# GewelsJI/MVLT

Measured on AMD Instinct MI355X. Metric: image-text pairs/sec/node, PVT-tiny MVLT pre-train step, higher is better.
Workload: dtype bf16

## Files before the change

### include/mvlt_hip.h

```cpp
#ifndef MVLT_HIP_H
#define MVLT_HIP_H
#include <stdint.h>
#ifdef __cplusplus
extern "C" {
#endif

#define MVLT_DT_BF16 0
#define MVLT_DT_FP32 1

#define MVLT_ABI_VERSION 8
const char* mvlt_last_error(void);
int mvlt_abi_version(void);
const char* mvlt_last_kernel(void);
int mvlt_sizeof(const char* name);

typedef struct mvlt_rowmap {
  int mode, rows_per_batch, batch_stride, offset;
  int r, w_in, tokens_in, hw_out, w_out, c_seg;
  int h_in;
} mvlt_rowmap;

typedef struct mvlt_gemm_nt_args {
  const void* A; const void* B; void* C;
  int M, N, K, lda, ldb, ldc;
// ... 163 lines not shown
  const void* residual;
  const float* row_scale; int rows_per_scale;
  void* out;
  void* h_out;
  float* dw1; float* db1; float* dw2; float* db2;
  int M, C, hid;
  const float* ln_x; const float* ln_gamma; const float* ln_beta; float ln_eps;
  void* ln_y; float* ln_mean; float* ln_rstd;
  void* out_op;
  const float* post_gamma; const float* post_beta; float post_eps;
  void* post_y; float* post_mean; float* post_rstd;
  const float* lnb_x; const float* lnb_mean; const float* lnb_rstd; const float* lnb_gamma;
  void* lnb_dx; void* lnb_dx2; const float* lnb_dx2_scale; int lnb_dx2_rows_per_scale;
  float* lnb_partials;
  void* partials; long partials_bytes; int defer_fold;
} mvlt_mlp_args;
int mvlt_mlp_fwd(const mvlt_mlp_args* args, void* stream);
int mvlt_mlp_bwd_dx(const mvlt_mlp_args* args, void* stream);
int mvlt_mlp_bwd_dw(const mvlt_mlp_args* args, void* stream);
int mvlt_add_column_sums(const float* in, long rows, int cols, int ld, float* dst0, int n0, float* dst1, void* stream);

int mvlt_col_stats(const float* z, int ldz, long M, int C, float* sum, float* sumsq, void* stream);
int mvlt_bn_finalize(const float* sum, const float* sumsq, int copies , long M, int C, float eps, float momentum, float* mean, float* rstd,
                     float* running_mean, float* running_var , void* stream);
int mvlt_bn_norm(const void* z, int ldz, int z_dtype, const float* mean, const float* rstd, const float* gamma, const float* beta, long M, int C,
                 void* y32, int ld32, int y32_dtype , void* y_op, int ld_op, int op_dtype , void* stream);
int mvlt_bn_finalize_norm(const void* z , int ldz, const float* sum, const float* sumsq, int copies, float eps, float momentum, float* mean, float* rstd,
                          float* running_mean, float* running_var , const float* gamma, const float* beta, long M, int C,
                          void* y32, int ld32, int y32_dtype, void* y_op , int ld_op, void* stream);
int mvlt_bn_bwd_reduce(const void* dy, int lddy, const void* z, int ldz, int z_dtype, const float* mean, const float* rstd, long M, int C,
// ... 21 lines not shown
```

### mvlt_amd/_lib.py

```python
import ctypes as C
import os

import torch

_HERE = os.path.dirname(os.path.abspath(__file__))
LIB_PATH = os.environ.get("MVLT_HIP_LIB") or os.path.join(_HERE, "libmvlt_hip.so")


class MVLTError(RuntimeError):
    pass


if not os.path.exists(LIB_PATH):
    raise ImportError(f"{LIB_PATH} is missing: build it with `python -m mvlt_amd.build` (hipcc, gfx950). "
                      "mvlt_amd has no CPU or eager fallback.")
lib = C.CDLL(LIB_PATH)

c_int, c_float, c_void_p, c_long = C.c_int, C.c_float, C.c_void_p, C.c_long


class RowMap(C.Structure):
    _fields_ = [(n, c_int) for n in ("mode", "rows_per_batch", "batch_stride", "offset",
                                     "r", "w_in", "tokens_in", "hw_out", "w_out", "c_seg", "h_in")]

# ... 58 lines not shown
                ("ldq", c_int), ("ldkv", c_int), ("ldo", c_int), ("lddkv", c_int),
                ("k_off", c_int), ("v_off", c_int), ("scale", c_float), ("dtype", c_int), ("dkv_dtype", c_int)]


class MlpArgs(C.Structure):
    _fields_ = [("x", c_void_p), ("dy", c_void_p), ("w1", c_void_p), ("wb", c_void_p), ("wc", c_void_p),
                ("b1", c_void_p), ("b2", c_void_p), ("residual", c_void_p), ("row_scale", c_void_p), ("rows_per_scale", c_int),
                ("out", c_void_p), ("h_out", c_void_p), ("dw1", c_void_p), ("db1", c_void_p), ("dw2", c_void_p), ("db2", c_void_p),
                ("M", c_int), ("C", c_int), ("hid", c_int),
                ("ln_x", c_void_p), ("ln_gamma", c_void_p), ("ln_beta", c_void_p), ("ln_eps", c_float),
                ("ln_y", c_void_p), ("ln_mean", c_void_p), ("ln_rstd", c_void_p), ("out_op", c_void_p),
                ("post_gamma", c_void_p), ("post_beta", c_void_p), ("post_eps", c_float),
                ("post_y", c_void_p), ("post_mean", c_void_p), ("post_rstd", c_void_p),
                ("lnb_x", c_void_p), ("lnb_mean", c_void_p), ("lnb_rstd", c_void_p), ("lnb_gamma", c_void_p),
                ("lnb_dx", c_void_p), ("lnb_dx2", c_void_p), ("lnb_dx2_scale", c_void_p), ("lnb_dx2_rows_per_scale", c_int),
                ("lnb_partials", c_void_p), ("partials", c_void_p), ("partials_bytes", c_long), ("defer_fold", c_int)]


STRUCTS = (("mvlt_rowmap", RowMap), ("mvlt_prep_desc", PrepDesc), ("mvlt_gemm_nt_args", GemmNTArgs), ("mvlt_gemm_tn_args", GemmTNArgs),
           ("mvlt_layernorm_args", LayerNormArgs), ("mvlt_layernorm_bwd_args", LayerNormBwdArgs),
           ("mvlt_attn_args", AttnArgs), ("mvlt_attn_bwd_args", AttnBwdArgs), ("mvlt_mlp_args", MlpArgs))

_vp, _i, _l, _f, _u64, _str = c_void_p, c_int, c_long, c_float, C.c_uint64, C.c_char_p
_by_args = lambda cls: (_i, [C.POINTER(cls), _vp])
PROTOTYPES = {
    "mvlt_last_error": (_str, []),
    "mvlt_abi_version": (_i, []),
    "mvlt_last_kernel": (_str, []),
    "mvlt_sizeof": (_i, [_str]),
    "mvlt_gemm_nt": _by_args(GemmNTArgs),
    "mvlt_gemm_tn": _by_args(GemmTNArgs),
# ... 132 lines not shown
```

### mvlt_amd/csrc/mlp.hip

```cpp
#include "common.h"
#include "../../include/mvlt_hip.h"
#include <type_traits>

namespace {

#ifndef MVLT_GELU_LUT
#define MVLT_GELU_LUT 1
#endif
#include "gelu_lut.inc"
constexpr int GELU_LUT_BYTES = MVLT_GELU_LUT_PAD * 8;
template <int NWV> __device__ __forceinline__ void gelu_lut_dma(unsigned lds_base, int wave, int lane) {
  for (int k = wave; k < GELU_LUT_BYTES / 1024; k += NWV)
    glds16((const char*)&g_gelu_lut[0][0] + k * 1024 + lane * 16, __builtin_amdgcn_readfirstlane(lds_base + k * 1024));
}
__device__ __forceinline__ unsigned gelu_lut_off(unsigned u) {
  return min(max(u, (unsigned)MVLT_GELU_LUT_BASE), (unsigned)MVLT_GELU_LUT_TOP) << 3;
}
__device__ __forceinline__ float gelu_lut_sign(float h) { return __builtin_bit_cast(float, (__builtin_bit_cast(unsigned, h) & 0x80000000u) | 0x3f800000u); }
template <int WHICH> __device__ __forceinline__ void gelu_lut_one2(const char* lut0, float h0, float h1, float& r0, float& r1) {
  const unsigned pk = __builtin_bit_cast(unsigned, __builtin_convertvector(f32x2{h0, h1}, bf16x2));
  const float t0 = *(const float*)(lut0 + gelu_lut_off(pk & 0x7fffu) + 4 * WHICH), t1 = *(const float*)(lut0 + gelu_lut_off((pk >> 16) & 0x7fffu) + 4 * WHICH);
  r0 = __builtin_fmaf(gelu_lut_sign(h0), t0, 0.5f);
  r1 = __builtin_fmaf(gelu_lut_sign(h1), t1, 0.5f);
}
// ... 5 lines not shown
  ph1 = __builtin_fmaf(s1, t1[0], 0.5f); d1 = __builtin_fmaf(s1, t1[1], 0.5f);
}

constexpr int NT = 256;
template <int C> struct MlpGeo { static constexpr int JC = (C == 64) ? 64 : 32; };

template <int K> __device__ __forceinline__ int toff(int row, int k) {
  constexpr int NCH = K / 8;
  int ch = k >> 3;
  int sw = (NCH == 4) ? (ch ^ ((row >> 2) & 3)) : (NCH == 8) ? (ch ^ ((row >> 1) & 7)) : (ch ^ (row & 15));
  return row * K + sw * 8 + (k & 7);
}

__device__ __forceinline__ bf16x8 ldfrag(const bf16* tile_base_elem) { return *(const bf16x8*)tile_base_elem; }

template <int C, int MODE>
__device__ __forceinline__ void mlp_load_rows(const mvlt_mlp_args& p, int m0, int wave, int fr, int fg, bf16x8 (&xfr)[2][C / 32],
                                              bf16x8 (&yfr)[MODE == 1 ? 2 : 1][C / 32]) {
  constexpr int MT = 2, WR = 32, KS_C = C / 32;
  const bf16* X = (const bf16*)p.x;
  const bf16* DY = (const bf16*)p.dy;
  if (MODE == 0 && p.ln_x) {
    const float inv_c = 1.0f / (float)C;
#pragma unroll
    for (int mt = 0; mt < MT; ++mt) {
      const int m = m0 + wave * WR + mt * 16 + fr;
      const bool ok = m < p.M;
      float v[KS_C][8];
      float sum = 0.f;
#pragma unroll
      for (int ks = 0; ks < KS_C; ++ks) {
        f32x4 a = {0.f, 0.f, 0.f, 0.f}, b = {0.f, 0.f, 0.f, 0.f};
        if (ok) {
          const float* src = p.ln_x + (long)m * C + ks * 32 + fg * 8;
          a = *(const f32x4*)src; b = *(const f32x4*)(src + 4);
        }
#pragma unroll
        for (int e = 0; e < 4; ++e) { v[ks][e] = a[e]; v[ks][4 + e] = b[e]; sum += a[e] + b[e]; }
      }
      sum += __shfl_xor(sum, 16); sum += __shfl_xor(sum, 32);
      const float mean = sum * inv_c;
      float q = 0.f;
#pragma unroll
      for (int ks = 0; ks < KS_C; ++ks)
#pragma unroll
        for (int e = 0; e < 8; ++e) { const float d = v[ks][e] - mean; q += d * d; }
      q += __shfl_xor(q, 16); q += __shfl_xor(q, 32);
      const float rstd = rsqrtf(q * inv_c + p.ln_eps);
      if (ok && fg == 0) { p.ln_mean[m] = mean; p.ln_rstd[m] = rstd; }
#pragma unroll
      for (int ks = 0; ks < KS_C; ++ks) {
        const float* gp = p.ln_gamma + ks * 32 + fg * 8;
        const float* bp = p.ln_beta + ks * 32 + fg * 8;
        const f32x4 g0 = *(const f32x4*)gp, g1 = *(const f32x4*)(gp + 4), be0 = *(const f32x4*)bp, be1 = *(const f32x4*)(bp + 4);
        bf16x8 o;
#pragma unroll
        for (int e = 0; e < 4; ++e) {
          o[e] = (bf16)((v[ks][e] - mean) * rstd * g0[e] + be0[e]);
          o[4 + e] = (bf16)((v[ks][4 + e] - mean) * rstd * g1[e] + be1[e]);
        }
        if (!ok) o = bf16x8{0, 0, 0, 0, 0, 0, 0, 0};
        xfr[mt][ks] = o;
        if (ok) st_g<MVLT_NT_MLP>((bf16x8*)((bf16*)p.ln_y + (long)m * C + ks * 32 + fg * 8), o);
      }
    }
  } else {
#pragma unroll
  for (int mt = 0; mt < MT; ++mt)
#pragma unroll
    for (int ks = 0; ks < KS_C; ++ks) {
      const int m = m0 + wave * WR + mt * 16 + fr;
      u32x4 v = {0u, 0u, 0u, 0u}, w = {0u, 0u, 0u, 0u};
      if (m < p.M) {
        v = *(const u32x4*)(X + (long)m * C + ks * 32 + fg * 8);
        if (MODE == 1) w = *(const u32x4*)(DY + (long)m * C + ks * 32 + fg * 8);
      }
      xfr[mt][ks] = __builtin_bit_cast(bf16x8, v);
      if (MODE == 1) yfr[mt][ks] = __builtin_bit_cast(bf16x8, w);
    }
  }
}

template <int C, int MODE, bool PFALL = true>
__device__ __forceinline__ void mlp_epilogue(const mvlt_mlp_args& p, char* smem, int m0, int tid, f32x4 (&oacc)[2][C / 16]) {
  constexpr int MT = 2, WR = 32, CT = C / 16;
  const int lane = tid & 63, wave = tid >> 6;
  const int fr = lane & 15, fg = lane >> 4;
  constexpr int LDW = C + 4, CPR = C / 8, RPI = 64 / CPR;
  float* stage = (float*)smem + wave * 16 * LDW;
  const int ch = lane % CPR;
  const int nc = ch * 8;
  float b2v[8];
#pragma unroll
  for (int e = 0; e < 8; ++e) b2v[e] = (MODE == 0) ? p.b2[nc + e] : 0.f;
  const bool lnb = MODE == 1 && p.lnb_x != nullptr;
// ... 296 lines not shown
#if MVLT_GELU_POLY & 1
  return gelu_poly_grad1(x);
#endif
  const float xc = __builtin_amdgcn_fmed3f(x, -7.0f, 7.0f);
  const float x2 = xc * xc;
  const float t = xc * __builtin_fmaf(__builtin_fmaf(x2, -MVLT_LOG2E * MVLT_GP2, -MVLT_LOG2E * MVLT_GP1), x2, -MVLT_LOG2E * MVLT_GP0);
  const float e = __builtin_amdgcn_exp2f(t);
  const float sg = __builtin_amdgcn_rcpf(e + 1.0f);
  const float up = __builtin_fmaf(__builtin_fmaf(x2, 5.0f * MVLT_GP2, 3.0f * MVLT_GP1), x2, MVLT_GP0);
  return __builtin_fmaf(x * up, sg * sg * e, sg);
}

#ifndef MVLT_PIPE_WAVES_64_1
#define MVLT_PIPE_WAVES_64_1 3
#endif
template <int C, int MODE>
__global__ __launch_bounds__(NT, (C == 64 && MODE == 1) ? MVLT_PIPE_WAVES_64_1 : 2) void mlp_pipe_kernel(mvlt_mlp_args p) {
  constexpr int MT = 2, CT = C / 16, KS_C = C / 32;
  constexpr int NP = MODE == 1 ? 2 : 1;
  constexpr int RB = 2 * C;
  constexpr int SPR = RB / 16;
  constexpr int RPI = 64 / SPR;
  constexpr int IPW = 32 / RPI / 4;
  constexpr int PB = 32 * RB;
  constexpr int CB = C * 64;
  constexpr int IPWC = C / 16 / 4;
  extern __shared__ __attribute__((aligned(16))) char smem[];
  char* const sP = smem;
  char* const sC = smem + 2 * NP * PB;
  float* const sB1 = (float*)(sC + 2 * CB);
  constexpr bool LUT = (MVLT_GELU_LUT >> (MODE == 1 ? 1 : 2)) & 1;
  const unsigned sP_lds = (unsigned)(uintptr_t)sP, sC_lds = (unsigned)(uintptr_t)sC;
// ... 25 lines not shown
      for (int it = 0; it < IPW; ++it)
        glds16(srcP[t][it] + so, __builtin_amdgcn_readfirstlane(sP_lds + (ring * NP + t) * PB + (wave + 4 * it) * 1024));
  };
  auto dmaC = [&](int u, int ring) {
#pragma unroll
    for (int it = 0; it < IPWC; ++it)
      glds16(srcC[it] + u * 64, __builtin_amdgcn_readfirstlane(sC_lds + ring * CB + (wave + 4 * it) * 1024));
  };
  dmaP(0, 0);
  if (NU > 1) dmaP(1, 1);
  const char* const lut0 = (const char*)(sB1 + hid) - 8 * MVLT_GELU_LUT_BASE;
  if (LUT) gelu_lut_dma<4>((unsigned)(uintptr_t)(sB1 + hid), wave, lane);
  for (int u = tid; u < hid; u += NT) sB1[u] = p.b1[u];

  bf16x8 xfr[MT][KS_C], yfr[MODE == 1 ? MT : 1][KS_C];
  mlp_load_rows<C, MODE>(p, m0, wave, fr, fg, xfr, yfr);

  const int rho0 = 8 * (fr >> 2) + (fr & 3);
  int poff[KS_C];
#pragma unroll
  for (int ks = 0; ks < KS_C; ++ks) poff[ks] = rho0 * RB + (((ks * 4 + fg) ^ pipe_fP<C>(rho0)) << 4);
  const int coff = fr * 64 + ((fg ^ pipe_gC(fr)) << 4);

  f32x4 oacc[MT][CT];
#pragma unroll
  for (int i = 0; i < MT; ++i)
#pragma unroll
    for (int j = 0; j < CT; ++j) oacc[i][j] = f32x4{0.f, 0.f, 0.f, 0.f};
  f32x4 hacc[2][2][MT], dgacc[MODE == 1 ? 2 : 1][2][MT];
  u32x4 gfrag[2][MT];

// ... 90 lines not shown
    dmaC(i, 1);
    iteration(P1{}, Y{}, Y{}, Y{}, i + 1);
    fence();
    dmaP(min(i + 3, NU - 1), 0);
    dmaC(i + 1, 0);
    iteration(P0{}, Y{}, Y{}, Y{}, i + 2);
    fence();
  }
  dmaC(NU - 1, 1);
  iteration(P1{}, N{}, Y{}, Y{}, 0);
  fence();
  iteration(P0{}, N{}, Y{}, N{}, 0);
  __syncthreads();
  mlp_epilogue<C, MODE, !(C == 64 && MODE == 1 && MVLT_PIPE_WAVES_64_1 >= 3)>(p, smem, m0, tid, oacc);
}

template <int C> __device__ __forceinline__ int wg_hs(int row) { return C == 64 ? ((row >> 1) & 3) : (row & 7); }

__device__ __forceinline__ float sload_f32(const float* ptr) {
  float v;
  asm volatile("s_load_dword %0, %1, 0x0\n\ts_waitcnt lgkmcnt(0)" : "=s"(v) : "s"(ptr) : "memory");
  return v;
}

template <int C>
__global__ __launch_bounds__(NT, C == 64 ? 2 : 1) void mlp_wgrad_kernel(mvlt_mlp_args p, int m_per_split, int splits, int ny) {
  constexpr int KS_C = C / 32, CT16 = C / 16;
  constexpr int ROWB = 2 * C;
  constexpr int CH = C / 8;
  constexpr int RPP = NT / CH;
// ... 521 lines not shown
  mvlt_max_lds<(mlp_wgrad_kernel<C>)>();
  MVLT_LAUNCH((mlp_wgrad_kernel<C>), dim3(8 * ((splits + 7) / 8) * ny), dim3(NT), lds, s, a, m_per_split, splits, ny);
  return mvlt_check_launch("mvlt_mlp_bwd_dw");
}

template <int C, int MODE> int launch(const mvlt_mlp_args& a, hipStream_t s) {
  constexpr int BM = 128, JC = MlpGeo<C>::JC;
  size_t lds = (size_t)(2 * JC * C * (MODE == 1 ? 2 : 1) + 2 * C * JC) * 2 + (size_t)a.hid * 4;
  if (MODE == 1 && ((MVLT_GELU_LUT >> 1) & 1)) lds += GELU_LUT_BYTES;
  const size_t stage = (size_t)4 * 16 * (C + 4) * 4;
  if (lds < stage) lds = stage;
  if (!a.h_out && a.hid >= 128) {
    size_t l2 = (size_t)2 * (MODE == 1 ? 2 : 1) * 32 * 2 * C + (size_t)2 * C * 64 + (size_t)a.hid * 4;
    if ((MVLT_GELU_LUT >> (MODE == 1 ? 1 : 2)) & 1) l2 += GELU_LUT_BYTES;
    if (l2 < stage) l2 = stage;
    mvlt_max_lds<(mlp_pipe_kernel<C, MODE>)>();
    MVLT_LAUNCH((mlp_pipe_kernel<C, MODE>), dim3((a.M + BM - 1) / BM), dim3(NT), l2, s, a);
    return mvlt_check_launch(MODE == 0 ? "mvlt_mlp_fwd" : "mvlt_mlp_bwd_dx");
  }
  mvlt_max_lds<(mlp_fused_kernel<C, MODE>)>();
  MVLT_LAUNCH((mlp_fused_kernel<C, MODE>), dim3((a.M + BM - 1) / BM), dim3(NT), lds, s, a);
  return mvlt_check_launch(MODE == 0 ? "mvlt_mlp_fwd" : "mvlt_mlp_bwd_dx");
}

int check(const mvlt_mlp_args* a, const char* who) {
  MVLT_REQUIRE(a && (a->x || a->ln_x) && a->w1 && a->wb && a->b1 && (a->out || a->out_op || a->lnb_x), "%s: null pointer", who);
  MVLT_REQUIRE(a->C == 64 || a->C == 128, "%s: C must be 64 or 128 (stage 1 / 2), got %d", who, a->C);
  MVLT_REQUIRE(a->hid > 0 && a->hid % 64 == 0, "%s: hidden size must be a multiple of 64", who);
  MVLT_REQUIRE(!a->row_scale || a->rows_per_scale > 0, "%s: row_scale needs rows_per_scale", who);
  return MVLT_OK;
}

}

extern "C" int mvlt_mlp_fwd(const mvlt_mlp_args* a, void* stream) {
  if (int e = check(a, "mvlt_mlp_fwd")) return e;
  MVLT_REQUIRE(a->b2 && a->residual, "mvlt_mlp_fwd: b2 and residual are required");
  MVLT_REQUIRE(!a->out_op || ((uintptr_t)a->out_op & 15) == 0, "mvlt_mlp_fwd: out_op must be 16-byte aligned");
  MVLT_REQUIRE(!a->post_y || (a->post_gamma && a->post_beta && a->post_mean && a->post_rstd && ((uintptr_t)a->post_y & 15) == 0),
               "mvlt_mlp_fwd: post_y needs post_gamma / post_beta / post_mean / post_rstd and 16-byte alignment");
  MVLT_REQUIRE(!a->ln_x || (a->ln_gamma && a->ln_beta && a->ln_y && a->ln_mean && a->ln_rstd && ((uintptr_t)a->ln_x & 15) == 0 && ((uintptr_t)a->ln_y & 15) == 0),
               "mvlt_mlp_fwd: the folded LayerNorm needs gamma, beta, y, mean, rstd and 16-byte aligned rows");
  if (a->M <= 0) return MVLT_OK;
  return a->C == 64 ? launch<64, 0>(*a, (hipStream_t)stream) : launch<128, 0>(*a, (hipStream_t)stream);
}

extern "C" int mvlt_mlp_bwd_dx(const mvlt_mlp_args* a, void* stream) {
  if (int e = check(a, "mvlt_mlp_bwd_dx")) return e;
  MVLT_REQUIRE(a->dy && a->wc, "mvlt_mlp_bwd_dx: dy and wc (W2^T) are required");
  MVLT_REQUIRE(!a->lnb_x || (a->lnb_mean && a->lnb_rstd && a->lnb_gamma && a->lnb_dx && a->lnb_partials && (!a->lnb_dx2 || (a->lnb_dx2_scale && a->lnb_dx2_rows_per_scale > 0)) &&
                             ((uintptr_t)a->lnb_x & 15) == 0 && ((uintptr_t)a->lnb_dx & 15) == 0 && ((uintptr_t)a->lnb_dx2 & 15) == 0),
               "mvlt_mlp_bwd_dx: lnb_x needs lnb_mean / lnb_rstd / lnb_gamma / lnb_dx / lnb_partials (and a scale for lnb_dx2), 16-byte aligned");
// ... 13 lines not shown
```

### mvlt_amd/ops.py

```python
import ctypes as C

import torch

from . import _lib as L
from ._lib import DT, check, patchmap, ptr, rowmap, stream_ptr

_ID = rowmap()


def gemm_nt(A, B, C_out, M, N, K, lda, ldb, ldc, *, a_map=None, c_map=None, bias=None, act=0, H=None,
            row_scale=None, rows_per_scale=0, R=None, col_sum=None, col_sumsq=None, col_copies=0, split_k=0, post_ln=None):
    assert A.dtype == B.dtype and A.dtype in DT and (C_out.dtype in DT or (C_out.dtype == torch.float16 and col_sum is not None))
    if bias is not None:
        assert bias.dtype == torch.float32
    if row_scale is not None:
        assert row_scale.dtype == torch.float32
    if R is not None:
        assert R.dtype == C_out.dtype or (R.dtype == torch.float32 and C_out.dtype == torch.bfloat16)
    if H is not None:
        assert H.dtype == C_out.dtype
    if col_sum is not None:
        assert col_sum.dtype == torch.float32 and col_sumsq is not None and col_sumsq.dtype == torch.float32
    a = L.GemmNTArgs(A=ptr(A), B=ptr(B), C=ptr(C_out), M=M, N=N, K=K, lda=lda, ldb=ldb, ldc=ldc,
                     dtype=DT[A.dtype], out_dtype=2 if C_out.dtype == torch.float16 else DT[C_out.dtype], a_map=a_map or _ID, c_map=c_map or _ID,
# ... 304 lines not shown
def upsample_l1_ok(W, scale):
    return W <= 64 and (W * scale) % 4 == 0 and W * scale <= 256


def upsample_l1_fwd(x, ldx, B, H, W, Cdim, scale, target, loss_sum):
    assert x.dtype == target.dtype == loss_sum.dtype == torch.float32 and target.is_contiguous()
    check(L.lib.mvlt_upsample_l1_fwd(ptr(x), ldx, B, H, W, Cdim, scale, ptr(target), ptr(loss_sum), stream_ptr()), "mvlt_upsample_l1_fwd")


def upsample_l1_bwd(x, ldx, B, H, W, Cdim, scale, target, gscale, dx, lddx):
    assert x.dtype == target.dtype == gscale.dtype == torch.float32 and dx.dtype in DT and target.is_contiguous()
    check(L.lib.mvlt_upsample_l1_bwd(ptr(x), ldx, B, H, W, Cdim, scale, ptr(target), ptr(gscale), ptr(dx), lddx, DT[dx.dtype], stream_ptr()),
          "mvlt_upsample_l1_bwd")


def mlp_fwd(x, w1, b1, w2, b2, residual, out, M, Cdim, hid, *, row_scale=None, rows_per_scale=0, h_out=None, ln=None, out_op=None, post_ln=None):
    assert w1.dtype == torch.bfloat16 and w2.dtype == torch.bfloat16
    assert residual.dtype == torch.float32 and residual.is_contiguous() and (out is not None or out_op is not None)
    assert out is None or out.dtype == torch.float32
    assert out_op is None or (out_op.dtype == torch.bfloat16 and out_op.is_contiguous())
    a = L.MlpArgs(x=ptr(x), w1=ptr(w1), wb=ptr(w2), b1=ptr(b1), b2=ptr(b2), residual=ptr(residual), row_scale=ptr(row_scale), rows_per_scale=rows_per_scale,
                  out=ptr(out), h_out=ptr(h_out), M=M, C=Cdim, hid=hid, out_op=ptr(out_op))
    if ln is None:
        assert x.dtype == torch.bfloat16
    else:
        g, b, eps, y, mean, rstd = ln
        assert g.dtype == b.dtype == mean.dtype == rstd.dtype == torch.float32 and y.dtype == torch.bfloat16 and y.is_contiguous()
        a.ln_x, a.ln_gamma, a.ln_beta, a.ln_eps, a.ln_y, a.ln_mean, a.ln_rstd = ptr(residual), ptr(g), ptr(b), eps, ptr(y), ptr(mean), ptr(rstd)
    if post_ln is not None:
        pg, pb, peps, py, pm, pr = post_ln
        assert pg.dtype == pb.dtype == pm.dtype == pr.dtype == torch.float32 and py.dtype == torch.bfloat16 and py.is_contiguous()
        a.post_gamma, a.post_beta, a.post_eps, a.post_y, a.post_mean, a.post_rstd = ptr(pg), ptr(pb), peps, ptr(py), ptr(pm), ptr(pr)
    check(L.lib.mvlt_mlp_fwd(C.byref(a), stream_ptr()), "mvlt_mlp_fwd")
    return out if out is not None else out_op


def mlp_bwd_dx(x, dy, w1, w1t, w2t, b1, out, M, Cdim, hid, *, row_scale=None, rows_per_scale=0, ln_bwd=None):
    assert x.dtype == dy.dtype == torch.bfloat16 and (out is None or out.dtype == torch.bfloat16)
    a = L.MlpArgs(x=ptr(x), dy=ptr(dy), w1=ptr(w1), wb=ptr(w1t), wc=ptr(w2t), b1=ptr(b1), row_scale=ptr(row_scale), rows_per_scale=rows_per_scale, M=M, C=Cdim, hid=hid)
    if ln_bwd is None:
# ... 98 lines not shown
```

### mvlt_amd/schedule.py

```python
import torch
import torch.nn.functional as F

from . import ops
from ._lib import patchmap, rowmap
from .params import ZeroPool, pool_zeros
from .pvlt import BERT_DROP, EPS_BERT, EPS_BLOCK, EPS_DEFAULT, VOCAB, VOCAB_LD


def _empty(shape, dtype, dev):
    return torch.empty(shape, dtype=dtype, device=dev)


def conv_wgrad(S, name, dz, xin, M, cout, K, ld_dz, ld_in, bmap, taps, cin, colsum=None):
    ops.gemm_tn(dz, xin, S.grad_taps(name, cout, taps, cin), M, cout, K, ld_dz, ld_in, K, b_map=bmap, colsum=colsum, partials=S.tn_partials(), defer_fold=True)


def _step_rng(model):
    model._rng_calls = getattr(model, "_rng_calls", 0) + 1
    return torch.initial_seed(), model._rng_calls


def check_input_size(model, Himg, Wimg):
    unit = model.patch_size * 8
    assert Himg % unit == 0 and Wimg % unit == 0, \
# ... 102 lines not shown
    units.append(PlanUnit("text_embeddings", "bert", dict(embed=[n for n in names if n.startswith("text_embeddings.")]), live))
    return BackwardPlan(units, live)


def _plan_for(model):
    S = model.store
    key = (id(S.P), tuple(p.requires_grad for p in S._plist))
    hit = getattr(S, "_plan", None)
    if hit is None or hit[0] != key:
        hit = S._plan = (key, backward_plan(model))
    return hit[1]


class TrunkStep:

    def __init__(self, model, images, ids, need_grad, plan=None):
        self.m = model
        self.S = model.store
        self.plan = plan if need_grad else None
        self.dev = images.device
        self.dt = model.compute_dtype
        self.rt = torch.float32
        self.need_grad = need_grad
        self.images = images.contiguous().float()
        self.ids = ids.contiguous()
        self.B = images.shape[0]
        assert images.shape[1] == model.in_chans
        Himg, Wimg = images.shape[2], images.shape[3]
        check_input_size(model, Himg, Wimg)
        self.Himg, self.Wimg = Himg, Wimg
        self.T = ids.shape[1]
        assert self.T == model.T_num, "input_ids length must equal num_text_tokens"
# ... 226 lines not shown
        else:
            Mk = N
            kv = _empty((B, Mk, 2 * C), dt, dev)
            ops.gemm_nt(xn1, self.w(p + "attn.kv.weight"), kv, M, 2 * C, C, C, C, 2 * C, bias=self.f32(p + "attn.kv.bias"))
        bs["kv"], bs["Mk"] = kv, Mk
        ao = _empty((B, N, C), dt, dev)
        lse = _empty((B, h, N), f32, dev)
        ops.sr_attention_fwd(q, kv, ao, lse, B, h, N, Mk, C, 2 * C, C, 0, C, 64 ** -0.5)
        bs["ao"], bs["lse"] = ao, lse
        xm = _empty((B, N, C), self.rt, dev)
        xn2 = _empty((B, N, C), dt, dev)
        bs["m2"], bs["r2"] = _empty((M,), f32, dev), _empty((M,), f32, dev)
        bs["xn2"] = xn2
        bs["fused_mlp"] = fused = (dt == torch.bfloat16 and C in (64, 128))
        proj_ln = fused and M < (1 << 24)
        ops.gemm_nt(ao, self.w(p + "attn.proj.weight"), xm, M, C, C, C, C, C, bias=self.f32(p + "attn.proj.bias"),
                    row_scale=s1, rows_per_scale=N, R=x,
                    post_ln=(self.f32(p + "norm2.weight"), self.f32(p + "norm2.bias"), EPS_BLOCK, xn2.view(M, C), bs["m2"], bs["r2"]) if proj_ln else None)
        bs["xm"] = xm
        last_op = fused and j == m.depths[i] - 1 and self.dt != self.rt
        last_gemm = ((not fused) and j == m.depths[i] - 1 and dt == torch.bfloat16 and self.rt == torch.float32 and
                     M < (1 << 24) and C % 8 == 0)
        xo = _empty((B, N, C), dt if (last_op or last_gemm) else self.rt, dev)
        if fused:
            ln = None if proj_ln else (self.f32(p + "norm2.weight"), self.f32(p + "norm2.bias"), EPS_BLOCK, xn2, bs["m2"], bs["r2"])
            post = None
            if j + 1 < m.depths[i]:
                pn = Names.blk(i, j + 1)
                self._pre_ln1 = (_empty((B, N, C), dt, dev), _empty((M,), f32, dev), _empty((M,), f32, dev))
                post = (self.f32(pn + "norm1.weight"), self.f32(pn + "norm1.bias"), EPS_BLOCK, *self._pre_ln1)
            ops.mlp_fwd(None if ln else xn2, self.w(p + "mlp.fc1.weight"), self.f32(p + "mlp.fc1.bias"), self.w(p + "mlp.fc2.weight"),
                        self.f32(p + "mlp.fc2.bias"), xm, None if last_op else xo, M, C, hid, row_scale=s2, rows_per_scale=N, ln=ln,
                        out_op=xo if last_op else None, post_ln=post)
        else:
            ops.layernorm_fwd(xm, xn2, self.f32(p + "norm2.weight"), self.f32(p + "norm2.bias"), M, C, C, C, EPS_BLOCK, mean=bs["m2"], rstd=bs["r2"])
            hpre = _empty((M, hid), dt, dev) if keep else None
            gact = _empty((M, hid), dt, dev)
            ops.gemm_nt(xn2, self.w(p + "mlp.fc1.weight"), gact, M, hid, C, C, C, hid, bias=self.f32(p + "mlp.fc1.bias"), act=1, H=hpre)
            bs["hpre"], bs["gact"] = hpre, gact
            ops.gemm_nt(gact, self.w(p + "mlp.fc2.weight"), xo, M, C, hid, hid, hid, C, bias=self.f32(p + "mlp.fc2.bias"),
                        row_scale=s2, rows_per_scale=N, R=xm)
        if not keep:
            bs.clear()
        return xo, bs

    def _scaled(self, dy, scale, N):
        if scale is None:
            return dy
# ... 209 lines not shown
            ops.gemm_nt(dkv, wkvT, dxn1, M, C, 2 * C, 2 * C, 2 * C, C, R=dxn1)
        prev = self.saved[i]["blocks"][j - 1] if j > 0 else None
        pre = prev is not None and not prev.get("fused_mlp", True) and prev.get("s2") is not None
        self._dy2_pre = _empty((M, C), dx.dtype, dev) if pre else None
        ops.layernorm_bwd(dxn1, bs["x"], dx, self.f32(p + "norm1.weight"), bs["m1"], bs["r1"], M, C, C, C, C,
                          dgamma=self.gl(p + "norm1.weight"), dbeta=self.gl(p + "norm1.bias"), **self.lnk(), accumulate=True,
                          dx2=self._dy2_pre, dx2_scale=prev["s2"] if pre else None, dx2_rows_per_scale=N if pre else 0, lddx2=C if pre else 0)
        bs.clear()
        return dx


class _TrunkFn(torch.autograd.Function):

    @staticmethod
    def forward(ctx, model, images, ids, need_grad, *params):
        step = TrunkStep(model, images, ids, need_grad, getattr(model, "_plan", None))
        outs = step.forward()
        ctx.step = step
        ctx.pool_token, model._pool_token = model._pool_token, None
        ctx.set_materialize_grads(False)
        ctx.mark_non_differentiable(outs[0])
        return tuple(outs)

    @staticmethod
    def backward(ctx, d1, d2, d3, d4):
        step = ctx.step
        S = step.S
        S.queue_finalize()
        step.backward([None, d2, d3, d4])
        ctx.step = None
        ctx.pool_token = None
# ... 352 lines not shown
```

Measured before the change: 13420.

## Fuse attention output projection and norm2 into the pipelined MLP forward kernel

Adds a projection prologue to the pipelined MLP forward kernel for stages with C=64/128. Each row block computes the attention proj GEMM with MFMA, adds bias, row scale and residual, writes xm, then runs LayerNorm in registers to produce the fc1 input. This removes a separate gemm_nt launch and the round trip of xn2 through memory. In exchange each wave reloads the CxC proj weight from global memory per output column group, occupancy changes, and the xn/mean/rstd stores are skipped when they are not kept for backward.

```diff
diff --git a/include/mvlt_hip.h b/include/mvlt_hip.h
--- a/include/mvlt_hip.h
+++ b/include/mvlt_hip.h
@@ -201,6 +201,10 @@
   void* lnb_dx; void* lnb_dx2; const float* lnb_dx2_scale; int lnb_dx2_rows_per_scale;
   float* lnb_partials;
   void* partials; long partials_bytes; int defer_fold;
+  const void* pj_ao; const void* pj_w; const float* pj_bias; const float* pj_x; const float* pj_scale;
+  float* pj_xm;
+  const float* pj_gamma; const float* pj_beta; float pj_eps;
+  void* pj_xn; float* pj_mean; float* pj_rstd;
 } mvlt_mlp_args;
 int mvlt_mlp_fwd(const mvlt_mlp_args* args, void* stream);
 int mvlt_mlp_bwd_dx(const mvlt_mlp_args* args, void* stream);
diff --git a/mvlt_amd/_lib.py b/mvlt_amd/_lib.py
--- a/mvlt_amd/_lib.py
+++ b/mvlt_amd/_lib.py
@@ -96,7 +96,9 @@
                 ("post_y", c_void_p), ("post_mean", c_void_p), ("post_rstd", c_void_p),
                 ("lnb_x", c_void_p), ("lnb_mean", c_void_p), ("lnb_rstd", c_void_p), ("lnb_gamma", c_void_p),
                 ("lnb_dx", c_void_p), ("lnb_dx2", c_void_p), ("lnb_dx2_scale", c_void_p), ("lnb_dx2_rows_per_scale", c_int),
-                ("lnb_partials", c_void_p), ("partials", c_void_p), ("partials_bytes", c_long), ("defer_fold", c_int)]
+                ("lnb_partials", c_void_p), ("partials", c_void_p), ("partials_bytes", c_long), ("defer_fold", c_int),
+                ("pj_ao", c_void_p), ("pj_w", c_void_p), ("pj_bias", c_void_p), ("pj_x", c_void_p), ("pj_scale", c_void_p), ("pj_xm", c_void_p),
+                ("pj_gamma", c_void_p), ("pj_beta", c_void_p), ("pj_eps", c_float), ("pj_xn", c_void_p), ("pj_mean", c_void_p), ("pj_rstd", c_void_p)]
 
 
 STRUCTS = (("mvlt_rowmap", RowMap), ("mvlt_prep_desc", PrepDesc), ("mvlt_gemm_nt_args", GemmNTArgs), ("mvlt_gemm_tn_args", GemmTNArgs),
diff --git a/mvlt_amd/csrc/mlp.hip b/mvlt_amd/csrc/mlp.hip
--- a/mvlt_amd/csrc/mlp.hip
+++ b/mvlt_amd/csrc/mlp.hip
@@ -43,6 +43,41 @@
 
 __device__ __forceinline__ bf16x8 ldfrag(const bf16* tile_base_elem) { return *(const bf16x8*)tile_base_elem; }
 
+template <int C, bool OPT>
+__device__ __forceinline__ void mlp_ln_row(const float (&v)[C / 32][8], float sum, bool ok, int m, int fg, const float* gamma, const float* beta, float eps,
+                                           bf16* y, float* mean_out, float* rstd_out, bf16x8 (&xf)[C / 32]) {
+  constexpr int KS_C = C / 32;
+  const float inv_c = 1.0f / (float)C;
+  sum += __shfl_xor(sum, 16); sum += __shfl_xor(sum, 32);
+  const float mean = sum * inv_c;
+  float q = 0.f;
+#pragma unroll
+  for (int ks = 0; ks < KS_C; ++ks)
+#pragma unroll
+    for (int e = 0; e < 8; ++e) { const float d = v[ks][e] - mean; q += d * d; }
+  q += __shfl_xor(q, 16); q += __shfl_xor(q, 32);
+  const float rstd = rsqrtf(q * inv_c + eps);
+  if (ok && fg == 0) {
+    if (!OPT || mean_out) mean_out[m] = mean;
+    if (!OPT || rstd_out) rstd_out[m] = rstd;
+  }
+#pragma unroll
+  for (int ks = 0; ks < KS_C; ++ks) {
+    const float* gp = gamma + ks * 32 + fg * 8;
+    const float* bp = beta + ks * 32 + fg * 8;
+    const f32x4 g0 = *(const f32x4*)gp, g1 = *(const f32x4*)(gp + 4), be0 = *(const f32x4*)bp, be1 = *(const f32x4*)(bp + 4);
+    bf16x8 o;
+#pragma unroll
+    for (int e = 0; e < 4; ++e) {
+      o[e] = (bf16)((v[ks][e] - mean) * rstd * g0[e] + be0[e]);
+      o[4 + e] = (bf16)((v[ks][4 + e] - mean) * rstd * g1[e] + be1[e]);
+    }
+    if (!ok) o = bf16x8{0, 0, 0, 0, 0, 0, 0, 0};
+    xf[ks] = o;
+    if (ok && (!OPT || y)) st_g<MVLT_NT_MLP>((bf16x8*)(y + (long)m * C + ks * 32 + fg * 8), o);
+  }
+}
+
 template <int C, int MODE>
 __device__ __forceinline__ void mlp_load_rows(const mvlt_mlp_args& p, int m0, int wave, int fr, int fg, bf16x8 (&xfr)[2][C / 32],
                                               bf16x8 (&yfr)[MODE == 1 ? 2 : 1][C / 32]) {
@@ -50,7 +85,6 @@
   const bf16* X = (const bf16*)p.x;
   const bf16* DY = (const bf16*)p.dy;
   if (MODE == 0 && p.ln_x) {
-    const float inv_c = 1.0f / (float)C;
 #pragma unroll
     for (int mt = 0; mt < MT; ++mt) {
       const int m = m0 + wave * WR + mt * 16 + fr;
@@ -67,31 +101,7 @@
 #pragma unroll
         for (int e = 0; e < 4; ++e) { v[ks][e] = a[e]; v[ks][4 + e] = b[e]; sum += a[e] + b[e]; }
       }
-      sum += __shfl_xor(sum, 16); sum += __shfl_xor(sum, 32);
-      const float mean = sum * inv_c;
-      float q = 0.f;
-#pragma unroll
-      for (int ks = 0; ks < KS_C; ++ks)
-#pragma unroll
-        for (int e = 0; e < 8; ++e) { const float d = v[ks][e] - mean; q += d * d; }
-      q += __shfl_xor(q, 16); q += __shfl_xor(q, 32);
-      const float rstd = rsqrtf(q * inv_c + p.ln_eps);
-      if (ok && fg == 0) { p.ln_mean[m] = mean; p.ln_rstd[m] = rstd; }
-#pragma unroll
-      for (int ks = 0; ks < KS_C; ++ks) {
-        const float* gp = p.ln_gamma + ks * 32 + fg * 8;
-        const float* bp = p.ln_beta + ks * 32 + fg * 8;
-        const f32x4 g0 = *(const f32x4*)gp, g1 = *(const f32x4*)(gp + 4), be0 = *(const f32x4*)bp, be1 = *(const f32x4*)(bp + 4);
-        bf16x8 o;
-#pragma unroll
-        for (int e = 0; e < 4; ++e) {
-          o[e] = (bf16)((v[ks][e] - mean) * rstd * g0[e] + be0[e]);
-          o[4 + e] = (bf16)((v[ks][4 + e] - mean) * rstd * g1[e] + be1[e]);
-        }
-        if (!ok) o = bf16x8{0, 0, 0, 0, 0, 0, 0, 0};
-        xfr[mt][ks] = o;
-        if (ok) st_g<MVLT_NT_MLP>((bf16x8*)((bf16*)p.ln_y + (long)m * C + ks * 32 + fg * 8), o);
-      }
+      mlp_ln_row<C, false>(v, sum, ok, m, fg, p.ln_gamma, p.ln_beta, p.ln_eps, (bf16*)p.ln_y, p.ln_mean, p.ln_rstd, xfr[mt]);
     }
   } else {
 #pragma unroll
@@ -108,6 +118,75 @@
       if (MODE == 1) yfr[mt][ks] = __builtin_bit_cast(bf16x8, w);
     }
   }
+}
+
+template <int C>
+__device__ __forceinline__ void mlp_proj_rows(const mvlt_mlp_args& p, int m0, int wave, int fr, int fg, bf16x8 (&xfr)[2][C / 32]) {
+  constexpr int MT = 2, WR = 32, KS_C = C / 32;
+  const bf16* AO = (const bf16*)p.pj_ao;
+  const bf16* WP = (const bf16*)p.pj_w;
+  constexpr int MTB = C == 64 ? 1 : 2;
+#pragma unroll
+  for (int mb = 0; mb < MT; mb += MTB) {
+    bf16x8 afr[MTB][KS_C];
+    float v[MTB][KS_C][8];
+    float rs[MTB];
+#pragma unroll
+    for (int t = 0; t < MTB; ++t) {
+      const int m = m0 + wave * WR + (mb + t) * 16 + fr;
+      const bool ok = m < p.M;
+      rs[t] = p.pj_scale ? p.pj_scale[(ok ? m : 0) / p.rows_per_scale] : 1.0f;
+#pragma unroll
+      for (int ks = 0; ks < KS_C; ++ks) {
+        u32x4 a = {0u, 0u, 0u, 0u};
+        f32x4 x0 = {0.f, 0.f, 0.f, 0.f}, x1 = {0.f, 0.f, 0.f, 0.f};
+        if (ok) {
+          a = *(const u32x4*)(AO + (long)m * C + ks * 32 + fg * 8);
+          const float* src = p.pj_x + (long)m * C + ks * 32 + fg * 8;
+          x0 = *(const f32x4*)src; x1 = *(const f32x4*)(src + 4);
+        }
+        afr[t][ks] = __builtin_bit_cast(bf16x8, a);
+#pragma unroll
+        for (int e = 0; e < 4; ++e) { v[t][ks][e] = x0[e]; v[t][ks][4 + e] = x1[e]; }
+      }
+    }
+#pragma unroll
+    for (int ks = 0; ks < KS_C; ++ks)
+#pragma unroll
+      for (int h = 0; h < 2; ++h) {
+        const int n = ks * 32 + 8 * (fr >> 2) + 4 * h + (fr & 3);
+        bf16x8 wf[KS_C];
+#pragma unroll
+        for (int kk = 0; kk < KS_C; ++kk) wf[kk] = *(const bf16x8*)(WP + n * C + kk * 32 + fg * 8);
+        const f32x4 bv = *(const f32x4*)(p.pj_bias + ks * 32 + 8 * fg + 4 * h);
+#pragma unroll
+        for (int t = 0; t < MTB; ++t) {
+          f32x4 acc = {0.f, 0.f, 0.f, 0.f};
+#pragma unroll
+          for (int kk = 0; kk < KS_C; ++kk) acc = __builtin_amdgcn_mfma_f32_16x16x32_bf16(wf[kk], afr[t][kk], acc, 0, 0, 0);
+#pragma unroll
+          for (int r = 0; r < 4; ++r) v[t][ks][4 * h + r] = (acc[r] + bv[r]) * rs[t] + v[t][ks][4 * h + r];
+        }
+      }
+#pragma unroll
+    for (int t = 0; t < MTB; ++t) {
+      const int m = m0 + wave * WR + (mb + t) * 16 + fr;
+      const bool ok = m < p.M;
+      float sum = 0.f;
+#pragma unroll
+      for (int ks = 0; ks < KS_C; ++ks) {
+#pragma unroll
+        for (int e = 0; e < 8; ++e) sum += v[t][ks][e];
+        if (ok) {
+          float* dst = p.pj_xm + (long)m * C + ks * 32 + fg * 8;
+          st_g<MVLT_NT_MLP>((f32x4*)dst, f32x4{v[t][ks][0], v[t][ks][1], v[t][ks][2], v[t][ks][3]});
+          st_g<MVLT_NT_MLP>((f32x4*)(dst + 4), f32x4{v[t][ks][4], v[t][ks][5], v[t][ks][6], v[t][ks][7]});
+        }
+      }
+      mlp_ln_row<C, true>(v[t], sum, ok, m, fg, p.pj_gamma, p.pj_beta, p.pj_eps, (bf16*)p.pj_xn, p.pj_mean, p.pj_rstd, xfr[mb + t]);
+    }
+  }
+  __builtin_amdgcn_fence(__ATOMIC_RELEASE, "wavefront");
 }
 
 template <int C, int MODE, bool PFALL = true>
@@ -434,8 +513,9 @@
 #ifndef MVLT_PIPE_WAVES_64_1
 #define MVLT_PIPE_WAVES_64_1 3
 #endif
-template <int C, int MODE>
-__global__ __launch_bounds__(NT, (C == 64 && MODE == 1) ? MVLT_PIPE_WAVES_64_1 : 2) void mlp_pipe_kernel(mvlt_mlp_args p) {
+template <int C, int MODE, bool PROJ>
+__device__ __forceinline__ void mlp_pipe_body(const mvlt_mlp_args& p) {
+  static_assert(!PROJ || MODE == 0, "the projection prologue belongs to the forward");
   constexpr int MT = 2, CT = C / 16, KS_C = C / 32;
   constexpr int NP = MODE == 1 ? 2 : 1;
   constexpr int RB = 2 * C;
@@ -491,7 +571,8 @@
   for (int u = tid; u < hid; u += NT) sB1[u] = p.b1[u];
 
   bf16x8 xfr[MT][KS_C], yfr[MODE == 1 ? MT : 1][KS_C];
-  mlp_load_rows<C, MODE>(p, m0, wave, fr, fg, xfr, yfr);
+  if constexpr (PROJ) mlp_proj_rows<C>(p, m0, wave, fr, fg, xfr);
+  else mlp_load_rows<C, MODE>(p, m0, wave, fr, fg, xfr, yfr);
 
   const int rho0 = 8 * (fr >> 2) + (fr & 3);
   int poff[KS_C];
@@ -612,6 +693,10 @@
   __syncthreads();
   mlp_epilogue<C, MODE, !(C == 64 && MODE == 1 && MVLT_PIPE_WAVES_64_1 >= 3)>(p, smem, m0, tid, oacc);
 }
+template <int C, int MODE>
+__global__ __launch_bounds__(NT, (C == 64 && MODE == 1) ? MVLT_PIPE_WAVES_64_1 : 2) void mlp_pipe_kernel(mvlt_mlp_args p) { mlp_pipe_body<C, MODE, false>(p); }
+template <int C>
+__global__ __launch_bounds__(NT, C == 64 ? 4 : 2) void mlp_pipe_proj_kernel(mvlt_mlp_args p) { mlp_pipe_body<C, 0, true>(p); }
 
 template <int C> __device__ __forceinline__ int wg_hs(int row) { return C == 64 ? ((row >> 1) & 3) : (row & 7); }
 
@@ -1163,6 +1248,15 @@
     size_t l2 = (size_t)2 * (MODE == 1 ? 2 : 1) * 32 * 2 * C + (size_t)2 * C * 64 + (size_t)a.hid * 4;
     if ((MVLT_GELU_LUT >> (MODE == 1 ? 1 : 2)) & 1) l2 += GELU_LUT_BYTES;
     if (l2 < stage) l2 = stage;
+    if constexpr (MODE == 0) {
+      if (a.pj_ao) {
+        mvlt_mlp_args b = a;
+        b.residual = a.pj_xm;
+        mvlt_max_lds<(mlp_pipe_proj_kernel<C>)>();
+        MVLT_LAUNCH((mlp_pipe_proj_kernel<C>), dim3((a.M + BM - 1) / BM), dim3(NT), l2, s, b);
+        return mvlt_check_launch("mvlt_mlp_fwd");
+      }
+    }
     mvlt_max_lds<(mlp_pipe_kernel<C, MODE>)>();
     MVLT_LAUNCH((mlp_pipe_kernel<C, MODE>), dim3((a.M + BM - 1) / BM), dim3(NT), l2, s, a);
     return mvlt_check_launch(MODE == 0 ? "mvlt_mlp_fwd" : "mvlt_mlp_bwd_dx");
@@ -1173,7 +1267,7 @@
 }
 
 int check(const mvlt_mlp_args* a, const char* who) {
-  MVLT_REQUIRE(a && (a->x || a->ln_x) && a->w1 && a->wb && a->b1 && (a->out || a->out_op || a->lnb_x), "%s: null pointer", who);
+  MVLT_REQUIRE(a && (a->x || a->ln_x || a->pj_ao) && a->w1 && a->wb && a->b1 && (a->out || a->out_op || a->lnb_x), "%s: null pointer", who);
   MVLT_REQUIRE(a->C == 64 || a->C == 128, "%s: C must be 64 or 128 (stage 1 / 2), got %d", who, a->C);
   MVLT_REQUIRE(a->hid > 0 && a->hid % 64 == 0, "%s: hidden size must be a multiple of 64", who);
   MVLT_REQUIRE(!a->row_scale || a->rows_per_scale > 0, "%s: row_scale needs rows_per_scale", who);
@@ -1184,7 +1278,13 @@
 
 extern "C" int mvlt_mlp_fwd(const mvlt_mlp_args* a, void* stream) {
   if (int e = check(a, "mvlt_mlp_fwd")) return e;
-  MVLT_REQUIRE(a->b2 && a->residual, "mvlt_mlp_fwd: b2 and residual are required");
+  MVLT_REQUIRE(a->b2 && (a->residual || a->pj_ao), "mvlt_mlp_fwd: b2 and residual are required");
+  if (a->pj_ao) {
+    MVLT_REQUIRE(a->pj_w && a->pj_bias && a->pj_x && a->pj_xm && a->pj_gamma && a->pj_beta, "mvlt_mlp_fwd: the projection prologue needs pj_w, pj_bias, pj_x, pj_xm, pj_gamma and pj_beta");
+    MVLT_REQUIRE(!a->ln_x && !a->h_out && a->hid >= 128, "mvlt_mlp_fwd: the projection prologue runs in the pipelined kernel only (no ln_x, no h_out, hid >= 128)");
+    MVLT_REQUIRE((((uintptr_t)a->pj_ao | (uintptr_t)a->pj_w | (uintptr_t)a->pj_bias | (uintptr_t)a->pj_x | (uintptr_t)a->pj_xm | (uintptr_t)a->pj_gamma | (uintptr_t)a->pj_beta |
+                   (uintptr_t)a->pj_xn) & 15) == 0, "mvlt_mlp_fwd: the projection prologue's tensors must be 16-byte aligned");
+  }
   MVLT_REQUIRE(!a->out_op || ((uintptr_t)a->out_op & 15) == 0, "mvlt_mlp_fwd: out_op must be 16-byte aligned");
   MVLT_REQUIRE(!a->post_y || (a->post_gamma && a->post_beta && a->post_mean && a->post_rstd && ((uintptr_t)a->post_y & 15) == 0),
                "mvlt_mlp_fwd: post_y needs post_gamma / post_beta / post_mean / post_rstd and 16-byte alignment");
diff --git a/mvlt_amd/ops.py b/mvlt_amd/ops.py
--- a/mvlt_amd/ops.py
+++ b/mvlt_amd/ops.py
@@ -342,16 +342,33 @@
           "mvlt_upsample_l1_bwd")
 
 
-def mlp_fwd(x, w1, b1, w2, b2, residual, out, M, Cdim, hid, *, row_scale=None, rows_per_scale=0, h_out=None, ln=None, out_op=None, post_ln=None):
+def mlp_fwd(x, w1, b1, w2, b2, residual, out, M, Cdim, hid, *, row_scale=None, rows_per_scale=0, h_out=None, ln=None, out_op=None, post_ln=None, proj=None):
     assert w1.dtype == torch.bfloat16 and w2.dtype == torch.bfloat16
-    assert residual.dtype == torch.float32 and residual.is_contiguous() and (out is not None or out_op is not None)
-    assert out is None or out.dtype == torch.float32
+    assert out is not None or out_op is not None
+    assert out is None or (out.dtype == torch.float32 and out.is_contiguous())
     assert out_op is None or (out_op.dtype == torch.bfloat16 and out_op.is_contiguous())
     a = L.MlpArgs(x=ptr(x), w1=ptr(w1), wb=ptr(w2), b1=ptr(b1), b2=ptr(b2), residual=ptr(residual), row_scale=ptr(row_scale), rows_per_scale=rows_per_scale,
                   out=ptr(out), h_out=ptr(h_out), M=M, C=Cdim, hid=hid, out_op=ptr(out_op))
-    if ln is None:
+    if proj is not None:
+        k = proj
+        assert x is None and residual is None and ln is None and h_out is None
+        assert k["ao"].dtype == k["w"].dtype == torch.bfloat16 and k["ao"].is_contiguous() and k["w"].is_contiguous() and tuple(k["w"].shape) == (Cdim, Cdim)
+        assert k["ao"].numel() == k["x"].numel() == M * Cdim and k["x"].dtype == torch.float32 and k["x"].is_contiguous()
+        assert k["bias"].dtype == k["gamma"].dtype == k["beta"].dtype == torch.float32 and k["bias"].numel() == k["gamma"].numel() == k["beta"].numel() == Cdim
+        scale, xm, xn, mean, rstd = k.get("scale"), k.get("xm"), k.get("xn"), k.get("mean"), k.get("rstd")
+        assert scale is None or (scale.dtype == torch.float32 and rows_per_scale > 0 and scale.numel() * rows_per_scale >= M)
+        assert xn is None or (xn.dtype == torch.bfloat16 and xn.is_contiguous() and xn.numel() == M * Cdim)
+        assert all(t is None or (t.dtype == torch.float32 and t.numel() == M) for t in (mean, rstd))
+        if xm is None:
+            xm = out if out is not None else torch.empty(M, Cdim, device=k["ao"].device, dtype=torch.float32)
+        assert xm.dtype == torch.float32 and xm.is_contiguous() and xm.numel() == M * Cdim
+        a.pj_ao, a.pj_w, a.pj_bias, a.pj_x, a.pj_scale, a.pj_xm = ptr(k["ao"]), ptr(k["w"]), ptr(k["bias"]), ptr(k["x"]), ptr(scale), ptr(xm)
+        a.pj_gamma, a.pj_beta, a.pj_eps, a.pj_xn, a.pj_mean, a.pj_rstd = ptr(k["gamma"]), ptr(k["beta"]), k["eps"], ptr(xn), ptr(mean), ptr(rstd)
+    else:
+        assert residual.dtype == torch.float32 and residual.is_contiguous()
+    if proj is None and ln is None:
         assert x.dtype == torch.bfloat16
-    else:
+    elif proj is None:
         g, b, eps, y, mean, rstd = ln
         assert g.dtype == b.dtype == mean.dtype == rstd.dtype == torch.float32 and y.dtype == torch.bfloat16 and y.is_contiguous()
         a.ln_x, a.ln_gamma, a.ln_beta, a.ln_eps, a.ln_y, a.ln_mean, a.ln_rstd = ptr(residual), ptr(g), ptr(b), eps, ptr(y), ptr(mean), ptr(rstd)
diff --git a/mvlt_amd/schedule.py b/mvlt_amd/schedule.py
--- a/mvlt_amd/schedule.py
+++ b/mvlt_amd/schedule.py
@@ -140,8 +140,9 @@
 
 class TrunkStep:
 
-    def __init__(self, model, images, ids, need_grad, plan=None):
+    def __init__(self, model, images, ids, need_grad, plan=None, proj_in_mlp=True):
         self.m = model
+        self.proj_in_mlp = proj_in_mlp
         self.S = model.store
         self.plan = plan if need_grad else None
         self.dev = images.device
@@ -398,9 +399,11 @@
         bs["xn2"] = xn2
         bs["fused_mlp"] = fused = (dt == torch.bfloat16 and C in (64, 128))
         proj_ln = fused and M < (1 << 24)
-        ops.gemm_nt(ao, self.w(p + "attn.proj.weight"), xm, M, C, C, C, C, C, bias=self.f32(p + "attn.proj.bias"),
-                    row_scale=s1, rows_per_scale=N, R=x,
-                    post_ln=(self.f32(p + "norm2.weight"), self.f32(p + "norm2.bias"), EPS_BLOCK, xn2.view(M, C), bs["m2"], bs["r2"]) if proj_ln else None)
+        proj_mlp = proj_ln and self.proj_in_mlp and hid >= 128 and x.dtype == f32
+        if not proj_mlp:
+            ops.gemm_nt(ao, self.w(p + "attn.proj.weight"), xm, M, C, C, C, C, C, bias=self.f32(p + "attn.proj.bias"),
+                        row_scale=s1, rows_per_scale=N, R=x,
+                        post_ln=(self.f32(p + "norm2.weight"), self.f32(p + "norm2.bias"), EPS_BLOCK, xn2.view(M, C), bs["m2"], bs["r2"]) if proj_ln else None)
         bs["xm"] = xm
         last_op = fused and j == m.depths[i] - 1 and self.dt != self.rt
         last_gemm = ((not fused) and j == m.depths[i] - 1 and dt == torch.bfloat16 and self.rt == torch.float32 and
@@ -413,9 +416,14 @@
                 pn = Names.blk(i, j + 1)
                 self._pre_ln1 = (_empty((B, N, C), dt, dev), _empty((M,), f32, dev), _empty((M,), f32, dev))
                 post = (self.f32(pn + "norm1.weight"), self.f32(pn + "norm1.bias"), EPS_BLOCK, *self._pre_ln1)
-            ops.mlp_fwd(None if ln else xn2, self.w(p + "mlp.fc1.weight"), self.f32(p + "mlp.fc1.bias"), self.w(p + "mlp.fc2.weight"),
-                        self.f32(p + "mlp.fc2.bias"), xm, None if last_op else xo, M, C, hid, row_scale=s2, rows_per_scale=N, ln=ln,
-                        out_op=xo if last_op else None, post_ln=post)
+            proj = None
+            if proj_mlp:
+                proj = dict(ao=ao, w=self.w(p + "attn.proj.weight"), bias=self.f32(p + "attn.proj.bias"), x=x, scale=s1, xm=xm,
+                            gamma=self.f32(p + "norm2.weight"), beta=self.f32(p + "norm2.bias"), eps=EPS_BLOCK,
+                            xn=xn2 if keep else None, mean=bs["m2"] if keep else None, rstd=bs["r2"] if keep else None)
+            ops.mlp_fwd(None if (ln or proj) else xn2, self.w(p + "mlp.fc1.weight"), self.f32(p + "mlp.fc1.bias"), self.w(p + "mlp.fc2.weight"),
+                        self.f32(p + "mlp.fc2.bias"), None if proj else xm, None if last_op else xo, M, C, hid, row_scale=s2, rows_per_scale=N, ln=ln,
+                        out_op=xo if last_op else None, post_ln=post, proj=proj)
         else:
             ops.layernorm_fwd(xm, xn2, self.f32(p + "norm2.weight"), self.f32(p + "norm2.bias"), M, C, C, C, EPS_BLOCK, mean=bs["m2"], rstd=bs["r2"])
             hpre = _empty((M, hid), dt, dev) if keep else None
@@ -655,7 +663,7 @@
 
     @staticmethod
     def forward(ctx, model, images, ids, need_grad, *params):
-        step = TrunkStep(model, images, ids, need_grad, getattr(model, "_plan", None))
+        step = TrunkStep(model, images, ids, need_grad, getattr(model, "_plan", None), proj_in_mlp=getattr(model, "_proj_in_mlp", True))
         outs = step.forward()
         ctx.step = step
         ctx.pool_token, model._pool_token = model._pool_token, None
```

New measurement: 13470 (median of 6 runs). No clear change (+0.3%).
